# senresearch/BulkLMM.jl

Hardware: AMD Instinct MI355X
Metric: trait x marker LOD tests/sec (higher is better)
Workload: dtype f64

## Files before the change

### bulklmm.jl_amd/csrc/kernels_scan.hip

```cpp
#include "blmm_internal.h"
#include "fastmath.h"
#include <type_traits>
#include <cmath>
#include <cstdlib>

namespace blmm {

#define KCHECK()                                                                                      \
  do {                                                                                                \
    hipError_t e__ = hipGetLastError();                                                               \
    if (e__ != hipSuccess) return fail(ctx, BLMM_ERR_HIP, std::string("kernel launch: ") + hipGetErrorString(e__)); \
  } while (0)

template <int N> struct VecD;
template <> struct VecD<1> { typedef double type; };
template <> struct VecD<2> { typedef double type __attribute__((ext_vector_type(2))); };
template <> struct VecD<4> { typedef double type __attribute__((ext_vector_type(4))); };

template <int N>
__device__ __forceinline__ void loadv(double (&dst)[N], const double* __restrict__ p) {
  if constexpr (N == 1) {
    dst[0] = p[0];
  } else if constexpr (N == 2) {
    const d2 v = *reinterpret_cast<const d2*>(p);
// ... 396 lines not shown
      else store_m<NB>(a.L + trait * a.ldL + i0, r, out, a.p - i0);
      if constexpr (PV) {
        double pv[NB];
#pragma unroll
        for (int nb = 0; nb < NB; ++nb) pv[nb] = fast_log10p1(out[nb], s_pv);
        store_m<NB>(a.Pv + trait * a.ldPv + i0, r, pv, a.p - i0);
      }
    }
  if (nnan) atomicAdd((unsigned long long*)&a.stat[ST_NAN_LOD], (unsigned long long)nnan);
  if constexpr (COND) {
    if (nrule) atomicAdd((unsigned long long*)&a.cinfo[0], (unsigned long long)nrule);
  }
}

template <int NX, bool TABLE, int MB, int W2 = 2, bool MORE = false>
static int launch_scan_t(blmm_ctx* ctx, const ScanArgs& a) {
  constexpr int NB = 4;
  static_assert(16 * W2 * MB <= 128 && 16 * W2 * NB <= TILE_I, "tile constants (operands are padded to 128)");
  const int64_t ntile_t = (a.m + 16 * W2 * MB - 1) / (16 * W2 * MB);
  const int64_t ntile_i = (a.p + 16 * W2 * NB - 1) / (16 * W2 * NB);
  const int64_t nwg = ntile_t * ntile_i;
  if (nwg <= 0) return BLMM_OK;
  if (nwg > 0x7fffffffLL) return fail(ctx, BLMM_ERR_INVALID, "problem too large for one launch");
  if (a.red.pmax) {
    if constexpr (TABLE && MB == 2 && W2 == 2 && !MORE)
      hipLaunchKernelGGL((k_scan<NX, MB, NB, TABLE, W2, false, MORE, false, true>), dim3((unsigned)nwg), dim3(64 * W2 * W2), 0, ctx->stream, a, (int)ntile_i, nwg);
    else
      return fail(ctx, BLMM_ERR_UNSUPPORTED, "reduce-in-epilogue: no such instantiation of k_scan");
  } else if (a.Pv)
    hipLaunchKernelGGL((k_scan<NX, MB, NB, TABLE, W2, false, MORE, true>), dim3((unsigned)nwg), dim3(64 * W2 * W2), 0, ctx->stream, a, (int)ntile_i, nwg);
  else
    hipLaunchKernelGGL((k_scan<NX, MB, NB, TABLE, W2, false, MORE>), dim3((unsigned)nwg), dim3(64 * W2 * W2), 0, ctx->stream, a, (int)ntile_i, nwg);
  KCHECK();
  return BLMM_OK;
}

int launch_scan_exact(blmm_ctx* ctx, const ScanArgs& a, int c) {
  switch (c) {
    case 1: {
      return launch_scan_t<2, false, 2, 2>(ctx, a);
    }
    case 2: return launch_scan_t<3, false, 1>(ctx, a);
    case 3: return launch_scan_t<4, false, 1>(ctx, a);
    case 4: return launch_scan_t<5, false, 1>(ctx, a);
  }
  if (c > CFAST && c <= CMAX && a.c == c) return launch_scan_t<1 + CFAST, false, 1, 2, true>(ctx, a);
  return fail(ctx, BLMM_ERR_UNSUPPORTED, BLMM_C_ERR);
}

template <int NX, int MB, bool MORE>
static int launch_scan_cond_t(blmm_ctx* ctx, const ScanArgs& a) {
  constexpr int NB = 4, W2 = 2;
  const int64_t ntile_t = (a.m + 16 * W2 * MB - 1) / (16 * W2 * MB);
  const int64_t ntile_i = (a.p + 16 * W2 * NB - 1) / (16 * W2 * NB);
  const int64_t nwg = ntile_t * ntile_i;
  if (nwg <= 0) return BLMM_OK;
  if (nwg > 0x7fffffffLL) return fail(ctx, BLMM_ERR_INVALID, "problem too large for one launch");
  if (a.red.pmax)
    hipLaunchKernelGGL((k_scan<NX, MB, NB, false, W2, false, MORE, false, true, true>), dim3((unsigned)nwg), dim3(64 * W2 * W2), 0, ctx->stream, a, (int)ntile_i, nwg);
  else
    hipLaunchKernelGGL((k_scan<NX, MB, NB, false, W2, false, MORE, false, false, true>), dim3((unsigned)nwg), dim3(64 * W2 * W2), 0, ctx->stream, a, (int)ntile_i, nwg);
  KCHECK();
  return BLMM_OK;
}

int launch_scan_cond(blmm_ctx* ctx, const ScanArgs& a, int ct) {
  if (!a.cflag || !a.cinfo || a.Pv || (a.red.pmax ? a.red.want_trip != 0 : !a.L) || a.c != ct)
    return fail(ctx, BLMM_ERR_INVALID, "launch_scan_cond: bad arguments");
  switch (ct) {
    case 1: return launch_scan_cond_t<2, 2, false>(ctx, a);
    case 2: return launch_scan_cond_t<3, 1, false>(ctx, a);
    case 3: return launch_scan_cond_t<4, 1, false>(ctx, a);
    case 4: return launch_scan_cond_t<5, 1, false>(ctx, a);
    case 5: case 6: case 7: case 8: return launch_scan_cond_t<1 + CFAST, 1, true>(ctx, a);
  }
  return fail(ctx, BLMM_ERR_UNSUPPORTED, "bulkscan_cond: 1 .. 8 null-design columns");
}

#ifdef LR_DIAG
__device__ unsigned long long g_lr_diag[24];
#endif
#ifdef LR_PHASE
__device__ unsigned long long g_lr_phase[8];
#endif
template <int C, int MB, int NB, bool PV = false, bool RED = false>
__global__ void __launch_bounds__(256, 2) k_scan_lr(LrArgs la, int ntile_i, int64_t nwg) {
  static_assert(!(RED && PV), "reduce-in-epilogue: no p-value output");
  const ScanArgs& a = la.s;
#ifdef LR_DIAG
  const unsigned long long diag_t0 = __builtin_amdgcn_s_memtime();
#endif
#ifdef LR_PHASE
  const unsigned long long ph_t0 = __builtin_amdgcn_s_memtime();
#endif
  constexpr int NACC = 2 + C;
  constexpr int NL = C * (C + 1) / 2;
  constexpr int TW = 32 * MB;
  __shared__ dpair s_lod[BLMM_LOD_TABLE_N];
  __shared__ double s_li[NL][TW];
  __shared__ int s_perm[TW];
  __shared__ dpair s_pv[PV ? BLMM_PV_TABLE_N * (BLMM_PV_STRIDE / 2) : 1];
  LodStage<256> lst;
  lod_stage_load<256>(lst, a.lodtab);
  const int lane = threadIdx.x & 63, wave = threadIdx.x >> 6;
  uint32_t tile_t; uint32_t tile_i;
  bool shared_w;
  {
    const uint32_t q = (uint32_t)(nwg >> 3);
    if (blockIdx.x >= (q << 3)) return;
    const uint32_t x = blockIdx.x & 7, local = blockIdx.x >> 3;
    const uint32_t nsh = (uint32_t)la.rg.counts[0], noth = (uint32_t)la.rg.counts[1];
    const uint32_t tb = (uint32_t)(la.rg.col0 / TW);
    const uint32_t ncolt = (uint32_t)(la.rg.ncol / TW);
    const uint32_t ns = (nsh + TW - 1) / TW, fo = ((uint32_t)la.rg.ncol - noth) / TW, nf = ncolt - fo;
    const uint64_t NS = la.skip_shared ? 0 : (uint64_t)ns * (uint32_t)ntile_i, NF = (uint64_t)nf * (uint32_t)ntile_i;
    const uint32_t sS = (uint32_t)((x * NS) >> 3), cS = (uint32_t)(((x + 1) * NS) >> 3) - sS;
    const uint32_t sF = (uint32_t)((x * NF) >> 3), cF = (uint32_t)(((x + 1) * NF) >> 3) - sF;
    if (local < cS) {
      shared_w = true;
      tile_of32(sS + local, ns, (uint32_t)ntile_i, tile_t, tile_i);
      tile_t += tb;
    } else if (local - cS < cF) {
      shared_w = false;
      tile_of32(sF + local - cS, nf, (uint32_t)ntile_i, tile_t, tile_i);
      tile_t += tb + fo;
    } else {
      return;
    }
  }
  static_assert(NL * TW <= 2 * 256, "L^-1 staging: two elements per thread");
  double li_st[2]; int perm_st = -1;
#pragma unroll
  for (int u = 0; u < 2; ++u) {
    const int e = (int)threadIdx.x + 256 * u;
    li_st[u] = (e < NL * TW) ? la.Ls[(int64_t)(e / TW) * a.ldp + (int64_t)tile_t * TW + (e % TW)] : 0.0;
  }
  if (threadIdx.x < TW) perm_st = la.perm[(int64_t)tile_t * TW + threadIdx.x];
  const int wt = wave >> 1, wi = wave & 1;
  const int64_t i0 = (int64_t)tile_i * (32 * NB) + wi * (16 * NB);
  const int r = lane & 15, kk = lane >> 4;

  const double* PA = a.P + (int64_t)tile_t * TW;
  const double* PB = a.Xt + (int64_t)tile_i * (32 * NB);
  const double* PC = la.Cp + (int64_t)tile_t * TW;
  int sgi = 0;
  if (la.seg.S > 1 && !shared_w)
    sgi = lr_seg_of(la.rg.ncol - 1 - ((int64_t)tile_t * TW - la.rg.col0), la.rg.segcnt, la.seg.S);
  const double* PT = la.T + (int64_t)sgi * (1 + C) * la.tstride + (int64_t)tile_i * (32 * NB);
  const uint32_t voffA = (uint32_t)(((int64_t)kk * a.ldp + wt * (16 * MB) + MB * r) * 8);
  const uint32_t voffB = (uint32_t)(((int64_t)kk * a.ldx + wi * (16 * NB)) * 8) + mvoff<NB>(r);
  const int64_t sa = 4 * a.ldp, sb = 4 * a.ldx;

  d4 acc[NACC][MB][NB];

  auto load1 = [&](double (&A)[2][MB], double (&B)[2][NB], int step2) {
#ifdef LR_NOLOAD
#pragma unroll
    for (int h = 0; h < 2; ++h) {
#pragma unroll
      for (int u = 0; u < MB; ++u) { A[h][u] = (double)(lane + step2 + u); asm volatile("" : "+v"(A[h][u])); }
#pragma unroll
      for (int u = 0; u < NB; ++u) { B[h][u] = (double)(lane - step2 + u); asm volatile("" : "+v"(B[h][u])); }
    }
    return;
#endif
#pragma unroll
// ... 125 lines not shown
#pragma unroll
      for (int reg = 0; reg < 4; ++reg) {
        const int64_t trait = s_perm[wt * (16 * MB) + MB * (kk + 4 * reg) + mb];
        if (trait < 0) continue;
        double li[NL];
        if constexpr (!SHW) {
#pragma unroll
          for (int e = 0; e < NL; ++e) li[e] = s_li[e][wt * (16 * MB) + MB * (kk + 4 * reg) + mb];
        }
        double uv[NB], out[NB];
#pragma unroll
        for (int nb = 0; nb < NB; ++nb) {
          const double num = acc[0][mb][nb][reg];
          double r2;
          if constexpr (SHW) {
            const double rr = num * rd[nb];
            r2 = rr * rr;
          } else {
            double xx = acc[1][mb][nb][reg];
#pragma unroll
            for (int q = 0; q < C; ++q) {
              double u = 0.0;
#pragma unroll
              for (int e = 0; e <= q; ++e) u = fma(li[q * (q + 1) / 2 + e], acc[2 + e][mb][nb][reg], u);
              xx = fma(-u, u, xx);
            }
            r2 = (num * num) * fast_rcp1(xx);
          }
          uv[nb] = 1.0 - r2;
        }
        bool ok = true;
#ifdef LR_NOEPI
#pragma unroll
        for (int nb = 0; nb < NB; ++nb) out[nb] = acc[0][mb][nb][reg] + acc[1][mb][nb][reg] + acc[2][mb][nb][reg];
#else
#pragma unroll
        for (int nb = 0; nb < NB; ++nb) { out[nb] = fast_lod5(uv[nb], s_lod, lp); ok = ok && lod_fast_ok(uv[nb]); }
        if (__builtin_expect(!ok, 0)) {
#pragma unroll
          for (int nb = 0; nb < NB; ++nb)
            if (!lod_fast_ok(uv[nb])) out[nb] = lod_out_of_range(uv[nb], s_lod, lp, scale, i0 + mslot<NB>(r, nb) < a.p, &nnan);
        }
#endif
#ifdef LR_NOSTORE
        if (out[0] + out[1] + out[2] + out[3] != 1.2345e-300) continue;
#endif
        if constexpr (RED) red_row<NB>(a.red, trait, i0, r, lane, out, red_valid(a.p, i0, 16 * NB));
        else store_m<NB>(a.L + trait * a.ldL + i0, r, out, a.p - i0);
        if constexpr (PV) {
          double pv[NB];
#pragma unroll
          for (int nb = 0; nb < NB; ++nb) pv[nb] = fast_log10p1(out[nb], s_pv);
          store_m<NB>(a.Pv + trait * a.ldPv + i0, r, pv, a.p - i0);
        }
      }
  };
  if (shared_w) epilogue(std::true_type{}); else epilogue(std::false_type{});
  if (nnan) atomicAdd((unsigned long long*)&a.stat[ST_NAN_LOD], (unsigned long long)nnan);
#ifdef LR_PHASE
  {
    __builtin_amdgcn_sched_barrier(0);
    const unsigned long long ph_t4 = __builtin_amdgcn_s_memtime();
    if (lane == 0) {
      unsigned long long* z = g_lr_phase + (shared_w ? 0 : 4);
      atomicAdd(&z[0], ph_t2 - ph_t0); atomicAdd(&z[1], ph_t3 - ph_t2); atomicAdd(&z[2], ph_t4 - ph_t3); atomicAdd(&z[3], 1ull);
    }
  }
#endif
#ifdef LR_DIAG
  if (threadIdx.x == 0) {
    atomicAdd(&g_lr_diag[shared_w ? 0 : 2], __builtin_amdgcn_s_memtime() - diag_t0);
    atomicAdd(&g_lr_diag[shared_w ? 1 : 3], 1ull);
    const unsigned xcc = __builtin_amdgcn_s_getreg(6164) & 15u;
    atomicMax(&g_lr_diag[8 + (xcc & 7)], __builtin_amdgcn_s_memrealtime());
    atomicAdd(&g_lr_diag[16 + (xcc & 7)], 1ull);
  }
#endif
}

template <int C, bool PV, bool RED = false>
__global__ void __launch_bounds__(256, 3) k_scan_lr3(LrArgs la, int ntile_i, int64_t nwg) {
  static_assert(!(RED && PV), "reduce-in-epilogue: no p-value output");
  const ScanArgs& a = la.s;
  constexpr int MB = 2, NB = 4, TW = 64;
  constexpr int NL = C * (C + 1) / 2;
  constexpr int NBC = (C == 1) ? 4 : 2;
  __shared__ dpair s_lod[BLMM_LOD_TABLE_N];
  __shared__ double s_li[NL][TW];
  __shared__ int s_perm[TW];
  __shared__ dpair s_pv[PV ? BLMM_PV_TABLE_N * (BLMM_PV_STRIDE / 2) : 1];
  LodStage<256> lst;
  lod_stage_load<256>(lst, a.lodtab);
  const int lane = threadIdx.x & 63, wave = threadIdx.x >> 6;
  uint32_t tile_t, tile_i;
  {
    const uint32_t q = (uint32_t)(nwg >> 3);
    if (blockIdx.x >= (q << 3)) return;
    const uint32_t x = blockIdx.x & 7, local = blockIdx.x >> 3;
    const uint32_t noth = (uint32_t)la.rg.counts[1];
    const uint32_t tb = (uint32_t)(la.rg.col0 / TW);
    const uint32_t ncolt = (uint32_t)(la.rg.ncol / TW);
    const uint32_t fo = ((uint32_t)la.rg.ncol - noth) / TW, nf = ncolt - fo;
    const uint64_t NF = (uint64_t)nf * (uint32_t)ntile_i;
    const uint32_t sF = (uint32_t)((x * NF) >> 3), cF = (uint32_t)(((x + 1) * NF) >> 3) - sF;
    if (local >= cF) return;
    tile_of32(sF + local, nf, (uint32_t)ntile_i, tile_t, tile_i);
    tile_t += tb + fo;
  }
  static_assert(NL * TW <= 2 * 256, "L^-1 staging: two elements per thread");
  double li_st[2]; int perm_st = -1;
#pragma unroll
  for (int u = 0; u < 2; ++u) {
    const int e = (int)threadIdx.x + 256 * u;
    li_st[u] = (e < NL * TW) ? la.Ls[(int64_t)(e / TW) * a.ldp + (int64_t)tile_t * TW + (e % TW)] : 0.0;
  }
  if (threadIdx.x < TW) perm_st = la.perm[(int64_t)tile_t * TW + threadIdx.x];
  const int wt = wave >> 1, wi = wave & 1;
  const int64_t i0 = (int64_t)tile_i * (32 * NB) + wi * (16 * NB);
  const int r = lane & 15, kk = lane >> 4;
  const double* PA = a.P + (int64_t)tile_t * TW;
  const double* PB = a.Xt + (int64_t)tile_i * (32 * NB);
  const double* PC = la.Cp + (int64_t)tile_t * TW;
  int sgi = 0;
  if (la.seg.S > 1) sgi = lr_seg_of(la.rg.ncol - 1 - ((int64_t)tile_t * TW - la.rg.col0), la.rg.segcnt, la.seg.S);
  const double* PT = la.T + (int64_t)sgi * (1 + C) * la.tstride + (int64_t)tile_i * (32 * NB);
  const uint32_t voffA = (uint32_t)(((int64_t)kk * a.ldp + wt * (16 * MB) + MB * r) * 8);
  const uint32_t voffB = (uint32_t)(((int64_t)kk * a.ldx + wi * (16 * NB)) * 8) + mvoff<NB>(r);
  const int64_t sa = 4 * a.ldp, sb = 4 * a.ldx;
  const int KR = la.rk[4 * sgi + 1];
  double c0[MB], d0[1 + C][NBC];
  auto load2 = [&](double (&A)[MB], double (&B)[1 + C][NBC], int step, int nb0) {
    bufload<MB>(A, make_srd(PC + (int64_t)step * sa), voffA);
#pragma unroll
    for (int q = 0; q <= C; ++q) bufload<NBC>(B[q], make_srd(PT + q * la.tstride + (int64_t)step * sb), voffB + (uint32_t)(8 * nb0));
  };
  if (KR > 0) load2(c0, d0, 0, 0);
  __builtin_amdgcn_sched_barrier(0);
  lod_stage_store<256>(lst, s_lod, a.lodc[0]);
#pragma unroll
  for (int u = 0; u < 2; ++u) {
    const int e = (int)threadIdx.x + 256 * u;
    if (e < NL * TW) s_li[e / TW][e % TW] = li_st[u];
  }
  if (threadIdx.x < TW) s_perm[threadIdx.x] = perm_st;
  if constexpr (PV) {
    const dpair* g = reinterpret_cast<const dpair*>(a.pvtab);
    for (int i = threadIdx.x; i < BLMM_PV_TABLE_N * (BLMM_PV_STRIDE / 2); i += 256) s_pv[i] = g[i];
  }
  __syncthreads();
  d4 den[MB][NB];
#pragma unroll
  for (int mb = 0; mb < MB; ++mb)
#pragma unroll
    for (int nb0 = 0; nb0 < NB; nb0 += NBC) {
      d4 sm[1 + C][NBC];
#pragma unroll
      for (int q = 0; q <= C; ++q)
#pragma unroll
        for (int nb = 0; nb < NBC; ++nb) sm[q][nb] = (d4){0, 0, 0, 0};
      for (int ks = 0; ks < KR; ++ks) {
        __builtin_amdgcn_sched_barrier(0);
#pragma unroll
        for (int nb = 0; nb < NBC; ++nb)
#pragma unroll
          for (int q = 0; q <= C; ++q) sm[q][nb] = __builtin_amdgcn_mfma_f64_16x16x4f64(c0[mb], d0[q][nb], sm[q][nb], 0, 0, 0);
        __builtin_amdgcn_sched_barrier(0);
        if (ks + 1 < KR) load2(c0, d0, ks + 1, nb0);
        else if (nb0 + NBC < NB) load2(c0, d0, 0, nb0 + NBC);
        else if (mb + 1 < MB) load2(c0, d0, 0, 0);
      }
#pragma unroll
      for (int reg = 0; reg < 4; ++reg) {
        double li[NL];
#pragma unroll
        for (int e = 0; e < NL; ++e) li[e] = s_li[e][wt * (16 * MB) + MB * (kk + 4 * reg) + mb];
#pragma unroll
        for (int nb = 0; nb < NBC; ++nb) {
          double xx = sm[0][nb][reg];
#pragma unroll
          for (int q = 0; q < C; ++q) {
            double u = 0.0;
#pragma unroll
            for (int e = 0; e <= q; ++e) u = fma(li[q * (q + 1) / 2 + e], sm[1 + e][nb][reg], u);
            xx = fma(-u, u, xx);
          }
          den[mb][nb0 + nb][reg] = fast_rcp1(xx);
        }
      }
#pragma unroll
      for (int nb = 0; nb < NBC; ++nb) asm volatile("" : "+v"(den[mb][nb0 + nb]));
    }
  d4 num[MB][NB];
#pragma unroll
  for (int mb = 0; mb < MB; ++mb)
#pragma unroll
    for (int nb = 0; nb < NB; ++nb) num[mb][nb] = (d4){0, 0, 0, 0};
  {
    double a0[MB], b0[NB];
    auto load1 = [&](double (&A)[MB], double (&B)[NB], int step) {
      bufload<MB>(A, make_srd(PA + (int64_t)step * sa), voffA);
      bufload_m<NB>(B, make_srd(PB + (int64_t)step * sb), voffB);
    };
    auto mf1 = [&](const double (&A)[MB], const double (&B)[NB]) {
#pragma unroll
      for (int mb = 0; mb < MB; ++mb)
#pragma unroll
        for (int nb = 0; nb < NB; ++nb) num[mb][nb] = __builtin_amdgcn_mfma_f64_16x16x4f64(A[mb], B[nb], num[mb][nb], 0, 0, 0);
    };
    const int K = a.ks;
    load1(a0, b0, 0);
    for (int s1 = 0; s1 < K; ++s1) {
      __builtin_amdgcn_sched_barrier(0);
      mf1(a0, b0);
      __builtin_amdgcn_sched_barrier(0);
      if (s1 + 1 < K) load1(a0, b0, s1 + 1);
    }
  }
  const double scale = a.lodc[0];
  const LodPoly5 lp = lod_poly5_of(a.lodc);
  int nnan = 0;
#pragma unroll
  for (int mb = 0; mb < MB; ++mb)
#pragma unroll
    for (int reg = 0; reg < 4; ++reg) {
      const int64_t trait = s_perm[wt * (16 * MB) + MB * (kk + 4 * reg) + mb];
      if (trait < 0) continue;
      double uv[NB], out[NB];
#pragma unroll
      for (int nb = 0; nb < NB; ++nb) {
        const double nm = num[mb][nb][reg];
        const double r2 = (nm * nm) * den[mb][nb][reg];
        uv[nb] = 1.0 - r2;
      }
      bool ok = true;
#pragma unroll
      for (int nb = 0; nb < NB; ++nb) { out[nb] = fast_lod5(uv[nb], s_lod, lp); ok = ok && lod_fast_ok(uv[nb]); }
      if (__builtin_expect(!ok, 0)) {
#pragma unroll
        for (int nb = 0; nb < NB; ++nb)
          if (!lod_fast_ok(uv[nb])) out[nb] = lod_out_of_range(uv[nb], s_lod, lp, scale, i0 + mslot<NB>(r, nb) < a.p, &nnan);
      }
      if constexpr (RED) red_row<NB>(a.red, trait, i0, r, lane, out, red_valid(a.p, i0, 16 * NB));
      else store_m<NB>(a.L + trait * a.ldL + i0, r, out, a.p - i0);
      if constexpr (PV) {
        double pv[NB];
#pragma unroll
        for (int nb = 0; nb < NB; ++nb) pv[nb] = fast_log10p1(out[nb], s_pv);
        store_m<NB>(a.Pv + trait * a.ldPv + i0, r, pv, a.p - i0);
      }
    }
  if (nnan) atomicAdd((unsigned long long*)&a.stat[ST_NAN_LOD], (unsigned long long)nnan);
}

template <int C, int MB>
static int launch_scan_lr_t(blmm_ctx* ctx, const LrArgs& la) {
  constexpr int NB = 4;
  const ScanArgs& a = la.s;
  const int64_t ntile_t = (a.m + 32 * MB - 1) / (32 * MB);
  const int64_t ntile_i = (a.p + 32 * NB - 1) / (32 * NB);
  if (ntile_t * ntile_i <= 0) return BLMM_OK;
  const int64_t nwg = (ntile_t * ntile_i + 16 + 7) / 8 * 8;
  if (nwg > 0x7fffffffLL) return fail(ctx, BLMM_ERR_INVALID, "problem too large for one launch");
#ifdef LR_DIAG
  unsigned long long z[24] = {0};
  (void)hipMemcpyToSymbol(HIP_SYMBOL(g_lr_diag), z, sizeof(z));
  (void)hipStreamSynchronize(ctx->stream);
#endif
#ifdef LR_PHASE
  unsigned long long zp[8] = {0};
  (void)hipMemcpyToSymbol(HIP_SYMBOL(g_lr_phase), zp, sizeof(zp));
  (void)hipStreamSynchronize(ctx->stream);
#endif
  static const bool lr3 = !(dev_env("BLMM_LR3") && dev_env("BLMM_LR3")[0] == '0');
  if (a.red.pmax && lr3 && C == 1 && MB == 2 && la.skip_shared && a.n <= 128)
    hipLaunchKernelGGL((k_scan_lr3<1, false, true>), dim3((unsigned)nwg), dim3(256), 0, ctx->stream, la, (int)ntile_i, nwg);
  else if (a.red.pmax)
    hipLaunchKernelGGL((k_scan_lr<C, MB, NB, false, true>), dim3((unsigned)nwg), dim3(256), 0, ctx->stream, la, (int)ntile_i, nwg);
  else if (a.Pv && lr3 && C == 1 && MB == 2 && la.skip_shared && a.n <= 128)
    hipLaunchKernelGGL((k_scan_lr3<1, true>), dim3((unsigned)nwg), dim3(256), 0, ctx->stream, la, (int)ntile_i, nwg);
  else if (a.Pv)
    hipLaunchKernelGGL((k_scan_lr<C, MB, NB, true>), dim3((unsigned)nwg), dim3(256), 0, ctx->stream, la, (int)ntile_i, nwg);
  else if (lr3 && C == 1 && MB == 2 && la.skip_shared && a.n <= 128)
    hipLaunchKernelGGL((k_scan_lr3<1, false>), dim3((unsigned)nwg), dim3(256), 0, ctx->stream, la, (int)ntile_i, nwg);
  else
    hipLaunchKernelGGL((k_scan_lr<C, MB, NB>), dim3((unsigned)nwg), dim3(256), 0, ctx->stream, la, (int)ntile_i, nwg);
#ifdef LR_PHASE
  (void)hipStreamSynchronize(ctx->stream);
  (void)hipMemcpyFromSymbol(zp, HIP_SYMBOL(g_lr_phase), sizeof(zp));
  for (int cls = 0; cls < 2; ++cls)
    if (zp[4 * cls + 3])
      fprintf(stderr, "lr phase: %s tiles: %llu waves, avg cycles K loops %.0f | barrier wait %.0f | epilogue %.0f\n", cls ? "rank-R" : "shared",
              zp[4 * cls + 3], (double)zp[4 * cls] / zp[4 * cls + 3], (double)zp[4 * cls + 1] / zp[4 * cls + 3], (double)zp[4 * cls + 2] / zp[4 * cls + 3]);
#endif
#ifdef LR_DIAG
  (void)hipStreamSynchronize(ctx->stream);
  (void)hipMemcpyFromSymbol(z, HIP_SYMBOL(g_lr_diag), sizeof(z));
  unsigned long long mn = ~0ull;
  for (int x = 0; x < 8; ++x) if (z[8 + x] && z[8 + x] < mn) mn = z[8 + x];
  fprintf(stderr, "lr diag: shared wgs %llu avg cycles %.0f | full wgs %llu avg cycles %.0f | xcd last-end ticks(100MHz) rel:", z[1],
          z[1] ? (double)z[0] / z[1] : 0.0, z[3], z[3] ? (double)z[2] / z[3] : 0.0);
  for (int x = 0; x < 8; ++x) fprintf(stderr, " %llu(%llu)", z[8 + x] - mn, z[16 + x]);
  fprintf(stderr, "\n");
#endif
  KCHECK();
  return BLMM_OK;
}

template <int C>
static bool lr3_covariates(blmm_ctx*, const LrArgs& la) {
  static const bool lr3 = !(dev_env("BLMM_LR3") && dev_env("BLMM_LR3")[0] == '0');
  return lr3 && la.skip_shared && la.s.n <= 128;
}
template <int C>
static int launch_scan_lr3_c(blmm_ctx* ctx, const LrArgs& la) {
  const ScanArgs& a = la.s;
  const int64_t ntile_t = (a.m + 63) / 64, ntile_i = (a.p + 127) / 128;
  if (ntile_t * ntile_i <= 0) return BLMM_OK;
  const int64_t nwg = (ntile_t * ntile_i + 16 + 7) / 8 * 8;
  if (nwg > 0x7fffffffLL) return fail(ctx, BLMM_ERR_INVALID, "problem too large for one launch");
  if (a.red.pmax) hipLaunchKernelGGL((k_scan_lr3<C, false, true>), dim3((unsigned)nwg), dim3(256), 0, ctx->stream, la, (int)ntile_i, nwg);
  else if (a.Pv) hipLaunchKernelGGL((k_scan_lr3<C, true>), dim3((unsigned)nwg), dim3(256), 0, ctx->stream, la, (int)ntile_i, nwg);
  else hipLaunchKernelGGL((k_scan_lr3<C, false>), dim3((unsigned)nwg), dim3(256), 0, ctx->stream, la, (int)ntile_i, nwg);
  KCHECK();
  return BLMM_OK;
}

int launch_scan_lr(blmm_ctx* ctx, const LrArgs& la) {
  switch (la.c) {
    case 1: {
      static const int mb1 = dev_env("BLMM_LR_MB1") ? atoi(dev_env("BLMM_LR_MB1")) : 0;
      return mb1 ? launch_scan_lr_t<1, 1>(ctx, la) : launch_scan_lr_t<1, 2>(ctx, la);
    }
    case 2: return lr3_covariates<2>(ctx, la) ? launch_scan_lr3_c<2>(ctx, la) : launch_scan_lr_t<2, 1>(ctx, la);
    case 3: return lr3_covariates<3>(ctx, la) ? launch_scan_lr3_c<3>(ctx, la) : launch_scan_lr_t<3, 1>(ctx, la);
  }
  return fail(ctx, BLMM_ERR_UNSUPPORTED, BLMM_C_ERR);
}

int launch_scan_shared(blmm_ctx* ctx, const ScanArgs& a) {
  constexpr int MB = 2, NB = 4, W2 = 2;
  const int64_t ntile_t = (a.m + 16 * W2 * MB - 1) / (16 * W2 * MB);
  const int64_t ntile_i = (a.p + 16 * W2 * NB - 1) / (16 * W2 * NB);
  if (ntile_t * ntile_i <= 0) return BLMM_OK;
  const int64_t nwg = (ntile_t * ntile_i + 8 + 7) / 8 * 8;
  if (nwg > 0x7fffffffLL) return fail(ctx, BLMM_ERR_INVALID, "problem too large for one launch");
  if (a.red.pmax)
    hipLaunchKernelGGL((k_scan<0, MB, NB, true, W2, true, false, false, true>), dim3((unsigned)nwg), dim3(64 * W2 * W2), 0, ctx->stream, a, (int)ntile_i, nwg);
  else if (a.Pv)
    hipLaunchKernelGGL((k_scan<0, MB, NB, true, W2, true, false, true>), dim3((unsigned)nwg), dim3(64 * W2 * W2), 0, ctx->stream, a, (int)ntile_i, nwg);
  else
    hipLaunchKernelGGL((k_scan<0, MB, NB, true, W2, true>), dim3((unsigned)nwg), dim3(64 * W2 * W2), 0, ctx->stream, a, (int)ntile_i, nwg);
  KCHECK();
  return BLMM_OK;
}

int launch_scan_table(blmm_ctx* ctx, const ScanArgs& a) {
  static const int mb = dev_env("BLMM_TABLE_MB") ? atoi(dev_env("BLMM_TABLE_MB")) : 2;
  if (mb == 4) return launch_scan_t<0, true, 4>(ctx, a);
  if (mb == 1) return launch_scan_t<0, true, 1>(ctx, a);
  return launch_scan_t<0, true, 2>(ctx, a);
}

#ifndef ALT_GT
#define ALT_GT 8
#endif
#ifndef ALT_MINW
#define ALT_MINW 3
#endif
template <int MB, int NB, bool BIDX8>
__global__ void __launch_bounds__(256, ALT_MINW) k_scan_alt(AltArgs aa, int ntile_i, int64_t nwg) {
  const ScanArgs& a = aa.s;
  __shared__ dpair s_lod[BLMM_LOD_TABLE_N];
  const double scale = a.lodc[0];
  {
    LodStage<256> lst;
    lod_stage_load<256>(lst, a.lodtab);
    lod_stage_store<256>(lst, s_lod, scale);
  }
  __syncthreads();
  const int lane = threadIdx.x & 63, wave = threadIdx.x >> 6;
  const uint32_t bid = (uint32_t)xcd_swizzle(blockIdx.x, nwg);
  uint32_t tile_t, tile_i;
  tile_of32<ALT_GT>(bid, (uint32_t)nwg / (uint32_t)ntile_i, (uint32_t)ntile_i, tile_t, tile_i);
  const int64_t t0 = (int64_t)tile_t * (32 * MB) + (wave >> 1) * (16 * MB);
  const int64_t i0 = (int64_t)tile_i * (32 * NB) + (wave & 1) * (16 * NB);
  const int r = lane & 15, kk = lane >> 4;
  const LodPoly5 lp = lod_poly5_of(a.lodc);

  static_assert(!BIDX8 || NB == 4, "packed arg-max: four outputs per register");
  double best[MB][NB][4];
  int bidx[MB][BIDX8 ? 1 : NB][4];
  d4 acc[MB][NB];
#pragma unroll
  for (int mb = 0; mb < MB; ++mb)
#pragma unroll
    for (int nb = 0; nb < NB; ++nb) {
      acc[mb][nb] = (d4){0, 0, 0, 0};
#pragma unroll
      for (int reg = 0; reg < 4; ++reg) { best[mb][nb][reg] = 0.0; bidx[mb][BIDX8 ? 0 : nb][reg] = 0; }
    }

  const double* PA = a.P + (int64_t)tile_t * (32 * MB);
  const double* PB = a.Xt + (int64_t)tile_i * (32 * NB);
  const uint32_t voffA = (uint32_t)(((int64_t)kk * a.ldp + (wave >> 1) * (16 * MB) + MB * r) * 8);
  const uint32_t voffB = (uint32_t)(((int64_t)kk * a.ldx + (wave & 1) * (16 * NB)) * 8) + mvoff<NB>(r);
// ... 146 lines not shown
```

Measured before the change: 167.1 billion.

## Reorder lr3 kernel: main GEMM first, per-mb denominator pass fused into epilogue

Restructures k_scan_lr3 so the numerator MFMA loop runs first, with double-buffered operand loads and the shared-memory staging overlapped with the first loads. The rank-R denominator GEMM and reciprocal are moved into the epilogue and done per mb row block, with a smaller NBC chunk. This is meant to cut live registers (den shrinks from MB*NB to NB vectors) and to hide load latency in the main loop. The cost is a serialized denominator pass per mb inside the epilogue. Also adds optional phase timing and trace instrumentation and factors the n<=128 limit into a constant.

New measurement: 166.9 billion. About the same (-0.1%).

```diff
diff --git a/bulklmm.jl_amd/csrc/kernels_scan.hip b/bulklmm.jl_amd/csrc/kernels_scan.hip
--- a/bulklmm.jl_amd/csrc/kernels_scan.hip
+++ b/bulklmm.jl_amd/csrc/kernels_scan.hip
@@ -793,9 +793,12 @@
 __global__ void __launch_bounds__(256, 3) k_scan_lr3(LrArgs la, int ntile_i, int64_t nwg) {
   static_assert(!(RED && PV), "reduce-in-epilogue: no p-value output");
   const ScanArgs& a = la.s;
+#ifdef LR_PHASE
+  const unsigned long long ph_t0 = __builtin_amdgcn_s_memtime();
+#endif
   constexpr int MB = 2, NB = 4, TW = 64;
   constexpr int NL = C * (C + 1) / 2;
-  constexpr int NBC = (C == 1) ? 4 : 2;
+  constexpr int NBC = (C == 1) ? 2 : 1;
   __shared__ dpair s_lod[BLMM_LOD_TABLE_N];
   __shared__ double s_li[NL][TW];
   __shared__ int s_perm[TW];
@@ -839,75 +842,18 @@
   const uint32_t voffB = (uint32_t)(((int64_t)kk * a.ldx + wi * (16 * NB)) * 8) + mvoff<NB>(r);
   const int64_t sa = 4 * a.ldp, sb = 4 * a.ldx;
   const int KR = la.rk[4 * sgi + 1];
-  double c0[MB], d0[1 + C][NBC];
-  auto load2 = [&](double (&A)[MB], double (&B)[1 + C][NBC], int step, int nb0) {
-    bufload<MB>(A, make_srd(PC + (int64_t)step * sa), voffA);
-#pragma unroll
-    for (int q = 0; q <= C; ++q) bufload<NBC>(B[q], make_srd(PT + q * la.tstride + (int64_t)step * sb), voffB + (uint32_t)(8 * nb0));
+  double c0, d0[1 + C][NBC];
+  auto load2 = [&](int step, int mb, int nb0) {
+    double A[1];
+    bufload<1>(A, make_srd(PC + (int64_t)step * sa), voffA + (uint32_t)(8 * mb));
+    c0 = A[0];
+#pragma unroll
+    for (int q = 0; q <= C; ++q) bufload<NBC>(d0[q], make_srd(PT + q * la.tstride + (int64_t)step * sb), voffB + (uint32_t)(8 * nb0));
   };
-  if (KR > 0) load2(c0, d0, 0, 0);
-  __builtin_amdgcn_sched_barrier(0);
-  lod_stage_store<256>(lst, s_lod, a.lodc[0]);
-#pragma unroll
-  for (int u = 0; u < 2; ++u) {
-    const int e = (int)threadIdx.x + 256 * u;
-    if (e < NL * TW) s_li[e / TW][e % TW] = li_st[u];
-  }
-  if (threadIdx.x < TW) s_perm[threadIdx.x] = perm_st;
-  if constexpr (PV) {
-    const dpair* g = reinterpret_cast<const dpair*>(a.pvtab);
-    for (int i = threadIdx.x; i < BLMM_PV_TABLE_N * (BLMM_PV_STRIDE / 2); i += 256) s_pv[i] = g[i];
-  }
-  __syncthreads();
-  d4 den[MB][NB];
-#pragma unroll
-  for (int mb = 0; mb < MB; ++mb)
-#pragma unroll
-    for (int nb0 = 0; nb0 < NB; nb0 += NBC) {
-      d4 sm[1 + C][NBC];
-#pragma unroll
-      for (int q = 0; q <= C; ++q)
-#pragma unroll
-        for (int nb = 0; nb < NBC; ++nb) sm[q][nb] = (d4){0, 0, 0, 0};
-      for (int ks = 0; ks < KR; ++ks) {
-        __builtin_amdgcn_sched_barrier(0);
-#pragma unroll
-        for (int nb = 0; nb < NBC; ++nb)
-#pragma unroll
-          for (int q = 0; q <= C; ++q) sm[q][nb] = __builtin_amdgcn_mfma_f64_16x16x4f64(c0[mb], d0[q][nb], sm[q][nb], 0, 0, 0);
-        __builtin_amdgcn_sched_barrier(0);
-        if (ks + 1 < KR) load2(c0, d0, ks + 1, nb0);
-        else if (nb0 + NBC < NB) load2(c0, d0, 0, nb0 + NBC);
-        else if (mb + 1 < MB) load2(c0, d0, 0, 0);
-      }
-#pragma unroll
-      for (int reg = 0; reg < 4; ++reg) {
-        double li[NL];
-#pragma unroll
-        for (int e = 0; e < NL; ++e) li[e] = s_li[e][wt * (16 * MB) + MB * (kk + 4 * reg) + mb];
-#pragma unroll
-        for (int nb = 0; nb < NBC; ++nb) {
-          double xx = sm[0][nb][reg];
-#pragma unroll
-          for (int q = 0; q < C; ++q) {
-            double u = 0.0;
-#pragma unroll
-            for (int e = 0; e <= q; ++e) u = fma(li[q * (q + 1) / 2 + e], sm[1 + e][nb][reg], u);
-            xx = fma(-u, u, xx);
-          }
-          den[mb][nb0 + nb][reg] = fast_rcp1(xx);
-        }
-      }
-#pragma unroll
-      for (int nb = 0; nb < NBC; ++nb) asm volatile("" : "+v"(den[mb][nb0 + nb]));
-    }
+
   d4 num[MB][NB];
-#pragma unroll
-  for (int mb = 0; mb < MB; ++mb)
-#pragma unroll
-    for (int nb = 0; nb < NB; ++nb) num[mb][nb] = (d4){0, 0, 0, 0};
   {
-    double a0[MB], b0[NB];
+    double a0[MB], b0[NB], a1[MB], b1[NB];
     auto load1 = [&](double (&A)[MB], double (&B)[NB], int step) {
       bufload<MB>(A, make_srd(PA + (int64_t)step * sa), voffA);
       bufload_m<NB>(B, make_srd(PB + (int64_t)step * sb), voffB);
@@ -918,20 +864,107 @@
 #pragma unroll
         for (int nb = 0; nb < NB; ++nb) num[mb][nb] = __builtin_amdgcn_mfma_f64_16x16x4f64(A[mb], B[nb], num[mb][nb], 0, 0, 0);
     };
+    load1(a0, b0, 0);
+    if (KR > 0) load2(0, 0, 0);
+    __builtin_amdgcn_sched_barrier(0);
+    lod_stage_store<256>(lst, s_lod, a.lodc[0]);
+#pragma unroll
+    for (int u = 0; u < 2; ++u) {
+      const int e = (int)threadIdx.x + 256 * u;
+      if (e < NL * TW) s_li[e / TW][e % TW] = li_st[u];
+    }
+    if (threadIdx.x < TW) s_perm[threadIdx.x] = perm_st;
+    if constexpr (PV) {
+      const dpair* g = reinterpret_cast<const dpair*>(a.pvtab);
+      for (int i = threadIdx.x; i < BLMM_PV_TABLE_N * (BLMM_PV_STRIDE / 2); i += 256) s_pv[i] = g[i];
+    }
+#pragma unroll
+    for (int mb = 0; mb < MB; ++mb)
+#pragma unroll
+      for (int nb = 0; nb < NB; ++nb) num[mb][nb] = (d4){0, 0, 0, 0};
+    __builtin_amdgcn_sched_barrier(0);
     const int K = a.ks;
-    load1(a0, b0, 0);
-    for (int s1 = 0; s1 < K; ++s1) {
+    int ks = 0;
+    for (; ks + 2 <= K; ks += 2) {
+      load1(a1, b1, ks + 1);
       __builtin_amdgcn_sched_barrier(0);
       mf1(a0, b0);
       __builtin_amdgcn_sched_barrier(0);
-      if (s1 + 1 < K) load1(a0, b0, s1 + 1);
-    }
-  }
+      load1(a0, b0, (ks + 2 < K) ? ks + 2 : ks);
+      __builtin_amdgcn_sched_barrier(0);
+      mf1(a1, b1);
+      __builtin_amdgcn_sched_barrier(0);
+    }
+    if (ks < K) mf1(a0, b0);
+  }
+#ifdef LR_PHASE
+  unsigned long long ph_k = __builtin_amdgcn_s_memtime() - ph_t0;
+  __builtin_amdgcn_sched_barrier(0);
+#endif
+  __syncthreads();
+#ifdef LR_PHASE
+  __builtin_amdgcn_sched_barrier(0);
+  const unsigned long long ph_t3 = __builtin_amdgcn_s_memtime();
+  const unsigned long long ph_bar = ph_t3 - ph_t0 - ph_k;
+  __builtin_amdgcn_sched_barrier(0);
+#endif
+
   const double scale = a.lodc[0];
   const LodPoly5 lp = lod_poly5_of(a.lodc);
   int nnan = 0;
-#pragma unroll
-  for (int mb = 0; mb < MB; ++mb)
+  const int vl = red_valid(a.p, i0, 16 * NB);
+#pragma unroll
+  for (int mb = 0; mb < MB; ++mb) {
+    d4 den[NB];
+#pragma unroll
+    for (int nb0 = 0; nb0 < NB; nb0 += NBC) {
+      d4 sm[1 + C][NBC];
+#pragma unroll
+      for (int q = 0; q <= C; ++q)
+#pragma unroll
+        for (int nb = 0; nb < NBC; ++nb) sm[q][nb] = (d4){0, 0, 0, 0};
+#ifdef LR_PHASE
+      __builtin_amdgcn_sched_barrier(0);
+      const unsigned long long ph_c0 = __builtin_amdgcn_s_memtime();
+#endif
+      for (int ks = 0; ks < KR; ++ks) {
+        __builtin_amdgcn_sched_barrier(0);
+#pragma unroll
+        for (int nb = 0; nb < NBC; ++nb)
+#pragma unroll
+          for (int q = 0; q <= C; ++q) sm[q][nb] = __builtin_amdgcn_mfma_f64_16x16x4f64(c0, d0[q][nb], sm[q][nb], 0, 0, 0);
+        __builtin_amdgcn_sched_barrier(0);
+        if (ks + 1 < KR) load2(ks + 1, mb, nb0);
+        else if (nb0 + NBC < NB) load2(0, mb, nb0 + NBC);
+        else if (mb + 1 < MB) load2(0, mb + 1, 0);
+      }
+#ifdef LR_PHASE
+      __builtin_amdgcn_sched_barrier(0);
+      ph_k += __builtin_amdgcn_s_memtime() - ph_c0;
+      __builtin_amdgcn_sched_barrier(0);
+#endif
+#pragma unroll
+      for (int reg = 0; reg < 4; ++reg) {
+        double li[NL];
+#pragma unroll
+        for (int e = 0; e < NL; ++e) li[e] = s_li[e][wt * (16 * MB) + MB * (kk + 4 * reg) + mb];
+#pragma unroll
+        for (int nb = 0; nb < NBC; ++nb) {
+          double xx = sm[0][nb][reg];
+#pragma unroll
+          for (int q = 0; q < C; ++q) {
+            double u = 0.0;
+#pragma unroll
+            for (int e = 0; e <= q; ++e) u = fma(li[q * (q + 1) / 2 + e], sm[1 + e][nb][reg], u);
+            xx = fma(-u, u, xx);
+          }
+          den[nb0 + nb][reg] = fast_rcp1(xx);
+        }
+        if constexpr (C > 1) __builtin_amdgcn_sched_barrier(0);
+      }
+#pragma unroll
+      for (int nb = 0; nb < NBC; ++nb) asm volatile("" : "+v"(den[nb0 + nb]));
+    }
 #pragma unroll
     for (int reg = 0; reg < 4; ++reg) {
       const int64_t trait = s_perm[wt * (16 * MB) + MB * (kk + 4 * reg) + mb];
@@ -940,18 +973,20 @@
 #pragma unroll
       for (int nb = 0; nb < NB; ++nb) {
         const double nm = num[mb][nb][reg];
-        const double r2 = (nm * nm) * den[mb][nb][reg];
+        const double r2 = (nm * nm) * den[nb][reg];
         uv[nb] = 1.0 - r2;
       }
       bool ok = true;
 #pragma unroll
       for (int nb = 0; nb < NB; ++nb) { out[nb] = fast_lod5(uv[nb], s_lod, lp); ok = ok && lod_fast_ok(uv[nb]); }
       if (__builtin_expect(!ok, 0)) {
+        double sc = scale;
+        asm volatile("" : "+v"(sc));
 #pragma unroll
         for (int nb = 0; nb < NB; ++nb)
-          if (!lod_fast_ok(uv[nb])) out[nb] = lod_out_of_range(uv[nb], s_lod, lp, scale, i0 + mslot<NB>(r, nb) < a.p, &nnan);
-      }
-      if constexpr (RED) red_row<NB>(a.red, trait, i0, r, lane, out, red_valid(a.p, i0, 16 * NB));
+          if (!lod_fast_ok(uv[nb])) out[nb] = lod_out_of_range(uv[nb], s_lod, lp, sc, mslot<NB>(r, nb) < vl, &nnan);
+      }
+      if constexpr (RED) red_row<NB>(a.red, trait, i0, r, lane, out, vl);
       else store_m<NB>(a.L + trait * a.ldL + i0, r, out, a.p - i0);
       if constexpr (PV) {
         double pv[NB];
@@ -960,9 +995,41 @@
         store_m<NB>(a.Pv + trait * a.ldPv + i0, r, pv, a.p - i0);
       }
     }
+  }
   if (nnan) atomicAdd((unsigned long long*)&a.stat[ST_NAN_LOD], (unsigned long long)nnan);
-}
-
+#ifdef LR_PHASE
+  {
+    __builtin_amdgcn_sched_barrier(0);
+    const unsigned long long ph_t4 = __builtin_amdgcn_s_memtime();
+    if (lane == 0) {
+      unsigned long long* z = g_lr_phase + 4;
+      atomicAdd(&z[0], ph_k); atomicAdd(&z[1], ph_bar); atomicAdd(&z[2], ph_t4 - ph_t0 - ph_k - ph_bar); atomicAdd(&z[3], 1ull);
+    }
+  }
+#endif
+}
+
+#ifdef LR_PHASE
+static void lr_phase_zero(blmm_ctx* ctx) {
+  unsigned long long zp[8] = {0};
+  (void)hipMemcpyToSymbol(HIP_SYMBOL(g_lr_phase), zp, sizeof(zp));
+  (void)hipStreamSynchronize(ctx->stream);
+}
+static void lr_phase_print(blmm_ctx* ctx) {
+  unsigned long long zp[8];
+  (void)hipStreamSynchronize(ctx->stream);
+  (void)hipMemcpyFromSymbol(zp, HIP_SYMBOL(g_lr_phase), sizeof(zp));
+  for (int cls = 0; cls < 2; ++cls)
+    if (zp[4 * cls + 3])
+      fprintf(stderr, "lr phase: %s tiles: %llu waves, avg cycles K loops %.0f | barrier wait %.0f | epilogue %.0f\n", cls ? "rank-R" : "shared",
+              zp[4 * cls + 3], (double)zp[4 * cls] / zp[4 * cls + 3], (double)zp[4 * cls + 1] / zp[4 * cls + 3], (double)zp[4 * cls + 2] / zp[4 * cls + 3]);
+}
+#endif
+static void lr_trace(const char* kernel, int c) {
+  static const bool on = dev_env("BLMM_LR_TRACE") && dev_env("BLMM_LR_TRACE")[0] == '1';
+  if (on) fprintf(stderr, "lr scan: %s c=%d\n", kernel, c);
+}
+constexpr int LR3_NMAX = 128;
 template <int C, int MB>
 static int launch_scan_lr_t(blmm_ctx* ctx, const LrArgs& la) {
   constexpr int NB = 4;
@@ -978,30 +1045,24 @@
   (void)hipStreamSynchronize(ctx->stream);
 #endif
 #ifdef LR_PHASE
-  unsigned long long zp[8] = {0};
-  (void)hipMemcpyToSymbol(HIP_SYMBOL(g_lr_phase), zp, sizeof(zp));
-  (void)hipStreamSynchronize(ctx->stream);
+  lr_phase_zero(ctx);
 #endif
   static const bool lr3 = !(dev_env("BLMM_LR3") && dev_env("BLMM_LR3")[0] == '0');
-  if (a.red.pmax && lr3 && C == 1 && MB == 2 && la.skip_shared && a.n <= 128)
+  lr_trace((lr3 && C == 1 && MB == 2 && la.skip_shared && a.n <= LR3_NMAX) ? "k_scan_lr3" : "k_scan_lr", C);
+  if (a.red.pmax && lr3 && C == 1 && MB == 2 && la.skip_shared && a.n <= LR3_NMAX)
     hipLaunchKernelGGL((k_scan_lr3<1, false, true>), dim3((unsigned)nwg), dim3(256), 0, ctx->stream, la, (int)ntile_i, nwg);
   else if (a.red.pmax)
     hipLaunchKernelGGL((k_scan_lr<C, MB, NB, false, true>), dim3((unsigned)nwg), dim3(256), 0, ctx->stream, la, (int)ntile_i, nwg);
-  else if (a.Pv && lr3 && C == 1 && MB == 2 && la.skip_shared && a.n <= 128)
+  else if (a.Pv && lr3 && C == 1 && MB == 2 && la.skip_shared && a.n <= LR3_NMAX)
     hipLaunchKernelGGL((k_scan_lr3<1, true>), dim3((unsigned)nwg), dim3(256), 0, ctx->stream, la, (int)ntile_i, nwg);
   else if (a.Pv)
     hipLaunchKernelGGL((k_scan_lr<C, MB, NB, true>), dim3((unsigned)nwg), dim3(256), 0, ctx->stream, la, (int)ntile_i, nwg);
-  else if (lr3 && C == 1 && MB == 2 && la.skip_shared && a.n <= 128)
+  else if (lr3 && C == 1 && MB == 2 && la.skip_shared && a.n <= LR3_NMAX)
     hipLaunchKernelGGL((k_scan_lr3<1, false>), dim3((unsigned)nwg), dim3(256), 0, ctx->stream, la, (int)ntile_i, nwg);
   else
     hipLaunchKernelGGL((k_scan_lr<C, MB, NB>), dim3((unsigned)nwg), dim3(256), 0, ctx->stream, la, (int)ntile_i, nwg);
 #ifdef LR_PHASE
-  (void)hipStreamSynchronize(ctx->stream);
-  (void)hipMemcpyFromSymbol(zp, HIP_SYMBOL(g_lr_phase), sizeof(zp));
-  for (int cls = 0; cls < 2; ++cls)
-    if (zp[4 * cls + 3])
-      fprintf(stderr, "lr phase: %s tiles: %llu waves, avg cycles K loops %.0f | barrier wait %.0f | epilogue %.0f\n", cls ? "rank-R" : "shared",
-              zp[4 * cls + 3], (double)zp[4 * cls] / zp[4 * cls + 3], (double)zp[4 * cls + 1] / zp[4 * cls + 3], (double)zp[4 * cls + 2] / zp[4 * cls + 3]);
+  lr_phase_print(ctx);
 #endif
 #ifdef LR_DIAG
   (void)hipStreamSynchronize(ctx->stream);
@@ -1020,7 +1081,7 @@
 template <int C>
 static bool lr3_covariates(blmm_ctx*, const LrArgs& la) {
   static const bool lr3 = !(dev_env("BLMM_LR3") && dev_env("BLMM_LR3")[0] == '0');
-  return lr3 && la.skip_shared && la.s.n <= 128;
+  return lr3 && la.skip_shared && la.s.n <= LR3_NMAX;
 }
 template <int C>
 static int launch_scan_lr3_c(blmm_ctx* ctx, const LrArgs& la) {
@@ -1029,9 +1090,16 @@
   if (ntile_t * ntile_i <= 0) return BLMM_OK;
   const int64_t nwg = (ntile_t * ntile_i + 16 + 7) / 8 * 8;
   if (nwg > 0x7fffffffLL) return fail(ctx, BLMM_ERR_INVALID, "problem too large for one launch");
+  lr_trace("k_scan_lr3", C);
+#ifdef LR_PHASE
+  lr_phase_zero(ctx);
+#endif
   if (a.red.pmax) hipLaunchKernelGGL((k_scan_lr3<C, false, true>), dim3((unsigned)nwg), dim3(256), 0, ctx->stream, la, (int)ntile_i, nwg);
   else if (a.Pv) hipLaunchKernelGGL((k_scan_lr3<C, true>), dim3((unsigned)nwg), dim3(256), 0, ctx->stream, la, (int)ntile_i, nwg);
   else hipLaunchKernelGGL((k_scan_lr3<C, false>), dim3((unsigned)nwg), dim3(256), 0, ctx->stream, la, (int)ntile_i, nwg);
+#ifdef LR_PHASE
+  lr_phase_print(ctx);
+#endif
   KCHECK();
   return BLMM_OK;
 }
```

## Interleave MFMA and buffer loads in lr3 K loops with split double-buffering

Applied to the files above, without the earlier changes.

Restructures both K loops of the lr3 scan kernel so that each MFMA group is immediately followed by the load of the next step's fragment for that group. The phase-2 covariate operand is double-buffered (cA/cB) and the phase-1 marker fragment is split into two 16-byte halves. The aim is to hide global load latency behind MFMA work and lower register pressure compared with loading whole fragments after all MFMAs finish. It also adds opt-in phase timers and a no-load diagnostic mode behind macros, plus a configurable n limit that defaults to the old value.

Measured after the change: 162.7 billion before, 166.6 billion after, median of 6. 2.4% higher.

```diff
diff --git a/bulklmm.jl_amd/csrc/kernels_scan.hip b/bulklmm.jl_amd/csrc/kernels_scan.hip
--- a/bulklmm.jl_amd/csrc/kernels_scan.hip
+++ b/bulklmm.jl_amd/csrc/kernels_scan.hip
@@ -502,6 +502,20 @@
 #endif
 #ifdef LR_PHASE
 __device__ unsigned long long g_lr_phase[8];
+__device__ unsigned long long g_lr3_phase[8];
+#define LR3_MARK(i)                                              \
+  {                                                              \
+    __builtin_amdgcn_sched_barrier(0);                           \
+    const unsigned long long t_ = __builtin_amdgcn_s_memtime();  \
+    ph_c[i] += t_ - ph_t;                                        \
+    ph_t = t_;                                                   \
+    __builtin_amdgcn_sched_barrier(0);                           \
+  }
+#else
+#define LR3_MARK(i)
+#endif
+#ifdef LR_NOLOAD
+__device__ __forceinline__ double lr3_regfed(double v) { asm volatile("" : "+v"(v)); return v; }
 #endif
 template <int C, int MB, int NB, bool PV = false, bool RED = false>
 __global__ void __launch_bounds__(256, 2) k_scan_lr(LrArgs la, int ntile_i, int64_t nwg) {
@@ -793,6 +807,10 @@
 __global__ void __launch_bounds__(256, 3) k_scan_lr3(LrArgs la, int ntile_i, int64_t nwg) {
   static_assert(!(RED && PV), "reduce-in-epilogue: no p-value output");
   const ScanArgs& a = la.s;
+#ifdef LR_PHASE
+  unsigned long long ph_c[5] = {0, 0, 0, 0, 0};
+  unsigned long long ph_t = __builtin_amdgcn_s_memtime();
+#endif
   constexpr int MB = 2, NB = 4, TW = 64;
   constexpr int NL = C * (C + 1) / 2;
   constexpr int NBC = (C == 1) ? 4 : 2;
@@ -839,13 +857,29 @@
   const uint32_t voffB = (uint32_t)(((int64_t)kk * a.ldx + wi * (16 * NB)) * 8) + mvoff<NB>(r);
   const int64_t sa = 4 * a.ldp, sb = 4 * a.ldx;
   const int KR = la.rk[4 * sgi + 1];
-  double c0[MB], d0[1 + C][NBC];
-  auto load2 = [&](double (&A)[MB], double (&B)[1 + C][NBC], int step, int nb0) {
-    bufload<MB>(A, make_srd(PC + (int64_t)step * sa), voffA);
-#pragma unroll
-    for (int q = 0; q <= C; ++q) bufload<NBC>(B[q], make_srd(PT + q * la.tstride + (int64_t)step * sb), voffB + (uint32_t)(8 * nb0));
+  double cA, cB, d0[1 + C][NBC];
+  auto ldc = [&](double& A, int step, int mb) {
+#ifdef LR_NOLOAD
+    A = lr3_regfed(1.0);
+    return;
+#endif
+    double t[1];
+    bufload<1>(t, make_srd(PC + (int64_t)step * sa), voffA + (uint32_t)(8 * mb));
+    A = t[0];
   };
-  if (KR > 0) load2(c0, d0, 0, 0);
+  auto ldd = [&](double (&B)[NBC], int q, int step, int nb0) {
+#ifdef LR_NOLOAD
+#pragma unroll
+    for (int u = 0; u < NBC; ++u) B[u] = lr3_regfed(q == 0 ? 1.0 : 1e-3 * (1 + ((lane + u + step + nb0) & 7)));
+    return;
+#endif
+    bufload<NBC>(B, make_srd(PT + q * la.tstride + (int64_t)step * sb), voffB + (uint32_t)(8 * nb0));
+  };
+  if (KR > 0) {
+    ldc(cA, 0, 0);
+#pragma unroll
+    for (int q = 0; q <= C; ++q) ldd(d0[q], q, 0, 0);
+  }
   __builtin_amdgcn_sched_barrier(0);
   lod_stage_store<256>(lst, s_lod, a.lodc[0]);
 #pragma unroll
@@ -859,6 +893,7 @@
     for (int i = threadIdx.x; i < BLMM_PV_TABLE_N * (BLMM_PV_STRIDE / 2); i += 256) s_pv[i] = g[i];
   }
   __syncthreads();
+  LR3_MARK(0)
   d4 den[MB][NB];
 #pragma unroll
   for (int mb = 0; mb < MB; ++mb)
@@ -869,17 +904,26 @@
       for (int q = 0; q <= C; ++q)
 #pragma unroll
         for (int nb = 0; nb < NBC; ++nb) sm[q][nb] = (d4){0, 0, 0, 0};
-      for (int ks = 0; ks < KR; ++ks) {
+      auto step2 = [&](bool more, int nstep, int nnb0, int nmb) {
         __builtin_amdgcn_sched_barrier(0);
-#pragma unroll
-        for (int nb = 0; nb < NBC; ++nb)
-#pragma unroll
-          for (int q = 0; q <= C; ++q) sm[q][nb] = __builtin_amdgcn_mfma_f64_16x16x4f64(c0[mb], d0[q][nb], sm[q][nb], 0, 0, 0);
+        if (more) ldc(cB, nstep, nmb);
         __builtin_amdgcn_sched_barrier(0);
-        if (ks + 1 < KR) load2(c0, d0, ks + 1, nb0);
-        else if (nb0 + NBC < NB) load2(c0, d0, 0, nb0 + NBC);
-        else if (mb + 1 < MB) load2(c0, d0, 0, 0);
-      }
+#pragma unroll
+        for (int q = 0; q <= C; ++q) {
+#pragma unroll
+          for (int nb = 0; nb < NBC; ++nb) sm[q][nb] = __builtin_amdgcn_mfma_f64_16x16x4f64(cA, d0[q][nb], sm[q][nb], 0, 0, 0);
+          __builtin_amdgcn_sched_barrier(0);
+          if (more) ldd(d0[q], q, nstep, nnb0);
+          __builtin_amdgcn_sched_barrier(0);
+        }
+      };
+      const bool samerow = nb0 + NBC < NB, nxc = samerow || mb + 1 < MB;
+      for (int ks = 0; ks + 1 < KR; ++ks) {
+        step2(true, ks + 1, nb0, mb);
+        cA = cB;
+      }
+      if (KR > 0) step2(nxc, 0, samerow ? nb0 + NBC : 0, samerow ? mb : mb + 1);
+      LR3_MARK(1)
 #pragma unroll
       for (int reg = 0; reg < 4; ++reg) {
         double li[NL];
@@ -900,6 +944,11 @@
       }
 #pragma unroll
       for (int nb = 0; nb < NBC; ++nb) asm volatile("" : "+v"(den[mb][nb0 + nb]));
+      if (nxc) {
+        __builtin_amdgcn_sched_barrier(0);
+        cA = cB;
+      }
+      LR3_MARK(2)
     }
   d4 num[MB][NB];
 #pragma unroll
@@ -907,26 +956,51 @@
 #pragma unroll
     for (int nb = 0; nb < NB; ++nb) num[mb][nb] = (d4){0, 0, 0, 0};
   {
-    double a0[MB], b0[NB];
-    auto load1 = [&](double (&A)[MB], double (&B)[NB], int step) {
+    static_assert(NB == 4, "phase 1: two 16-byte halves of the marker fragment");
+    double aA[MB], aB[MB], b0[2][2];
+    auto lda = [&](double (&A)[MB], int step) {
+#ifdef LR_NOLOAD
+#pragma unroll
+      for (int u = 0; u < MB; ++u) A[u] = lr3_regfed(0.05);
+      return;
+#endif
       bufload<MB>(A, make_srd(PA + (int64_t)step * sa), voffA);
-      bufload_m<NB>(B, make_srd(PB + (int64_t)step * sb), voffB);
     };
-    auto mf1 = [&](const double (&A)[MB], const double (&B)[NB]) {
-#pragma unroll
-      for (int mb = 0; mb < MB; ++mb)
-#pragma unroll
-        for (int nb = 0; nb < NB; ++nb) num[mb][nb] = __builtin_amdgcn_mfma_f64_16x16x4f64(A[mb], B[nb], num[mb][nb], 0, 0, 0);
+    auto ldb = [&](double (&B)[2], int step, int h) {
+#ifdef LR_NOLOAD
+#pragma unroll
+      for (int u = 0; u < 2; ++u) B[u] = lr3_regfed(0.03 * ((lane + u + 2 * h + step) & 15));
+      return;
+#endif
+      bufload<2>(B, make_srd(PB + (int64_t)step * sb), voffB + (uint32_t)(16 * h));
+    };
+    auto step1 = [&](bool more, int nstep) {
+      __builtin_amdgcn_sched_barrier(0);
+      if (more) lda(aB, nstep);
+      __builtin_amdgcn_sched_barrier(0);
+#pragma unroll
+      for (int h = 0; h < 2; ++h) {
+#pragma unroll
+        for (int nb = 2 * h; nb < 2 * h + 2; ++nb)
+#pragma unroll
+          for (int mb = 0; mb < MB; ++mb) num[mb][nb] = __builtin_amdgcn_mfma_f64_16x16x4f64(aA[mb], b0[h][nb - 2 * h], num[mb][nb], 0, 0, 0);
+        __builtin_amdgcn_sched_barrier(0);
+        if (more) ldb(b0[h], nstep, h);
+        __builtin_amdgcn_sched_barrier(0);
+      }
     };
     const int K = a.ks;
-    load1(a0, b0, 0);
-    for (int s1 = 0; s1 < K; ++s1) {
-      __builtin_amdgcn_sched_barrier(0);
-      mf1(a0, b0);
-      __builtin_amdgcn_sched_barrier(0);
-      if (s1 + 1 < K) load1(a0, b0, s1 + 1);
-    }
-  }
+    lda(aA, 0);
+    ldb(b0[0], 0, 0);
+    ldb(b0[1], 0, 1);
+    for (int s1 = 0; s1 + 1 < K; ++s1) {
+      step1(true, s1 + 1);
+#pragma unroll
+      for (int mb = 0; mb < MB; ++mb) aA[mb] = aB[mb];
+    }
+    if (K > 0) step1(false, 0);
+  }
+  LR3_MARK(3)
   const double scale = a.lodc[0];
   const LodPoly5 lp = lod_poly5_of(a.lodc);
   int nnan = 0;
@@ -961,7 +1035,35 @@
       }
     }
   if (nnan) atomicAdd((unsigned long long*)&a.stat[ST_NAN_LOD], (unsigned long long)nnan);
-}
+#ifdef LR_PHASE
+  LR3_MARK(4)
+  if (lane == 0) {
+#pragma unroll
+    for (int i = 0; i < 5; ++i) atomicAdd(&g_lr3_phase[i], ph_c[i]);
+    atomicAdd(&g_lr3_phase[5], 1ull);
+  }
+#endif
+}
+
+#ifdef LR_PHASE
+static void lr3_phase_reset(blmm_ctx* ctx) {
+  unsigned long long z[8] = {0};
+  (void)hipMemcpyToSymbol(HIP_SYMBOL(g_lr3_phase), z, sizeof(z));
+  (void)hipStreamSynchronize(ctx->stream);
+}
+static void lr3_phase_print(blmm_ctx* ctx) {
+  unsigned long long z[8];
+  (void)hipStreamSynchronize(ctx->stream);
+  (void)hipMemcpyFromSymbol(z, HIP_SYMBOL(g_lr3_phase), sizeof(z));
+  if (z[5])
+    fprintf(stderr, "lr3 phase: %llu waves, avg cycles head %.0f | phase-2 loops %.0f | conversions %.0f | phase-1 loop %.0f | epilogue %.0f\n", z[5],
+            (double)z[0] / z[5], (double)z[1] / z[5], (double)z[2] / z[5], (double)z[3] / z[5], (double)z[4] / z[5]);
+}
+#endif
+
+#ifndef LR3_NMAX
+#define LR3_NMAX 128
+#endif
 
 template <int C, int MB>
 static int launch_scan_lr_t(blmm_ctx* ctx, const LrArgs& la) {
@@ -981,17 +1083,18 @@
   unsigned long long zp[8] = {0};
   (void)hipMemcpyToSymbol(HIP_SYMBOL(g_lr_phase), zp, sizeof(zp));
   (void)hipStreamSynchronize(ctx->stream);
+  lr3_phase_reset(ctx);
 #endif
   static const bool lr3 = !(dev_env("BLMM_LR3") && dev_env("BLMM_LR3")[0] == '0');
-  if (a.red.pmax && lr3 && C == 1 && MB == 2 && la.skip_shared && a.n <= 128)
+  if (a.red.pmax && lr3 && C == 1 && MB == 2 && la.skip_shared && a.n <= LR3_NMAX)
     hipLaunchKernelGGL((k_scan_lr3<1, false, true>), dim3((unsigned)nwg), dim3(256), 0, ctx->stream, la, (int)ntile_i, nwg);
   else if (a.red.pmax)
     hipLaunchKernelGGL((k_scan_lr<C, MB, NB, false, true>), dim3((unsigned)nwg), dim3(256), 0, ctx->stream, la, (int)ntile_i, nwg);
-  else if (a.Pv && lr3 && C == 1 && MB == 2 && la.skip_shared && a.n <= 128)
+  else if (a.Pv && lr3 && C == 1 && MB == 2 && la.skip_shared && a.n <= LR3_NMAX)
     hipLaunchKernelGGL((k_scan_lr3<1, true>), dim3((unsigned)nwg), dim3(256), 0, ctx->stream, la, (int)ntile_i, nwg);
   else if (a.Pv)
     hipLaunchKernelGGL((k_scan_lr<C, MB, NB, true>), dim3((unsigned)nwg), dim3(256), 0, ctx->stream, la, (int)ntile_i, nwg);
-  else if (lr3 && C == 1 && MB == 2 && la.skip_shared && a.n <= 128)
+  else if (lr3 && C == 1 && MB == 2 && la.skip_shared && a.n <= LR3_NMAX)
     hipLaunchKernelGGL((k_scan_lr3<1, false>), dim3((unsigned)nwg), dim3(256), 0, ctx->stream, la, (int)ntile_i, nwg);
   else
     hipLaunchKernelGGL((k_scan_lr<C, MB, NB>), dim3((unsigned)nwg), dim3(256), 0, ctx->stream, la, (int)ntile_i, nwg);
@@ -1002,6 +1105,7 @@
     if (zp[4 * cls + 3])
       fprintf(stderr, "lr phase: %s tiles: %llu waves, avg cycles K loops %.0f | barrier wait %.0f | epilogue %.0f\n", cls ? "rank-R" : "shared",
               zp[4 * cls + 3], (double)zp[4 * cls] / zp[4 * cls + 3], (double)zp[4 * cls + 1] / zp[4 * cls + 3], (double)zp[4 * cls + 2] / zp[4 * cls + 3]);
+  lr3_phase_print(ctx);
 #endif
 #ifdef LR_DIAG
   (void)hipStreamSynchronize(ctx->stream);
@@ -1020,7 +1124,7 @@
 template <int C>
 static bool lr3_covariates(blmm_ctx*, const LrArgs& la) {
   static const bool lr3 = !(dev_env("BLMM_LR3") && dev_env("BLMM_LR3")[0] == '0');
-  return lr3 && la.skip_shared && la.s.n <= 128;
+  return lr3 && la.skip_shared && la.s.n <= LR3_NMAX;
 }
 template <int C>
 static int launch_scan_lr3_c(blmm_ctx* ctx, const LrArgs& la) {
@@ -1029,9 +1133,15 @@
   if (ntile_t * ntile_i <= 0) return BLMM_OK;
   const int64_t nwg = (ntile_t * ntile_i + 16 + 7) / 8 * 8;
   if (nwg > 0x7fffffffLL) return fail(ctx, BLMM_ERR_INVALID, "problem too large for one launch");
+#ifdef LR_PHASE
+  lr3_phase_reset(ctx);
+#endif
   if (a.red.pmax) hipLaunchKernelGGL((k_scan_lr3<C, false, true>), dim3((unsigned)nwg), dim3(256), 0, ctx->stream, la, (int)ntile_i, nwg);
   else if (a.Pv) hipLaunchKernelGGL((k_scan_lr3<C, true>), dim3((unsigned)nwg), dim3(256), 0, ctx->stream, la, (int)ntile_i, nwg);
   else hipLaunchKernelGGL((k_scan_lr3<C, false>), dim3((unsigned)nwg), dim3(256), 0, ctx->stream, la, (int)ntile_i, nwg);
+#ifdef LR_PHASE
+  lr3_phase_print(ctx);
+#endif
   KCHECK();
   return BLMM_OK;
 }
```
